# kento/TEZip

Measured on AMD Instinct MI355X. Metric: frames/sec (predict+delta-encode), 512x512 seq, higher is better.
Workload: dtype f32; 1 GPU; 512x512x3 synthetic turbulence stack, 80 frames per GPU (ONE 80-frame sequence), SWP 20-frame windows, warm_up 0, lossy rel 1e-3, entropy remap on; PredNet (3,48,96,192) glorot seed 123

## Files before the change

### tezip_amd/csrc/tz_conv_kernels.hip.h

```cpp
#pragma once
#include <type_traits>

#include "tz_internal.h"
#include "tz_math.hip.h"

typedef float f32x4 __attribute__((ext_vector_type(4)));

enum { EPI_RAW = 0, EPI_RELU = 1, EPI_LSTM = 2, EPI_LSTM_PACKED = 3, EPI_POOL_ERR = 4, EPI_LSTM3 = 5, EPI_RAW3 = 6 };

struct ConvSrc {
    const float* p;
    long long nstride;
    int C;
    int pstride;
    int up;
    int cpt;
};

struct ConvArgs {
    ConvSrc src[2];
    int nsrc;
    int H, W, tiles_x, tiles_y, ncb;
    const float* Wp;
    const float* Wimg;
// ... 1150 lines not shown

    __builtin_amdgcn_s_setprio(1);
    wait_vm_n(inflight);
    wg_barrier();
    {
        const float* pa = smem;
        const float* wb = smem + P0 * 256 + lane * NTI;
#pragma unroll
        for (int tap = 0; tap < 9; ++tap) {
            const int dy = tap / 3, dx = tap % 3;
            const int xo = MAP == MAP_PARITY ? (dx == 1 ? ((wcls & 1) ? 1 - PW / 2 : PW / 2) : (dx >> 1)) : dx;
            const int toff = 4 * (dy * PW + xo);
#pragma unroll
            for (int kk = 0; kk < KS0; ++kk) {
                float fa[MT];
#pragma unroll
                for (int mt = 0; mt < MT; ++mt) fa[mt] = pa[abase[mt] + toff + kk * 4 * NP16];
                mfma_step(fa, wb + (tap * KS0 + kk) * 64 * NTI);
            }
        }
    }
    if (UPS) {
#pragma unroll 1
        for (int b = 1; b < nblk; ++b) {
            if (b + 1 < nblk) {
                wg_barrier();
                inflight = issue_block(b + 1, (b + 1) & 1);
            } else {
                inflight = 0;
            }
            wait_vm_n(inflight);
            wg_barrier();
            const float* pa = smem + (b & 1) * BUFP * 256;
            const float* wb = pa + U16_PIECES * 256 + lane * NTI;
#pragma unroll
            for (int tap = 0; tap < 4; ++tap) {
                const int toff = 4 * ((tap >> 1) * LW + (tap & 1));
#pragma unroll
                for (int kk = 0; kk < 4; ++kk) {
                    float fa[MT];
#pragma unroll
                    for (int mt = 0; mt < MT; ++mt) fa[mt] = pa[abase_lo[mt] + toff + kk * 4 * NPU16];
                    mfma_step(fa, wb + ((tap * 4 + wcls) * 4 + kk) * 64 * NTI);
                }
            }
        }
    }
    __builtin_amdgcn_s_setprio(0);
    if (EPI == EPI_LSTM_PACKED) wg_barrier();
    if (EPI == EPI_POOL_ERR && a.dead_half) conv_epilogue<NT, EPI, MAP, true>(a, acc, n, cb, ty0, tx0, wv, lane, smem);
    else conv_epilogue<NT, EPI, MAP>(a, acc, n, cb, ty0, tx0, wv, lane, smem);
}

template <int CIN, int COUT>
__global__ __launch_bounds__(256) void k_conv_small(const ConvArgs a) {
    __shared__ float tile[PPIX * CIN];
    const int tid = threadIdx.x;
    const int ntiles = a.tiles_x * a.tiles_y;
    const int tileid = blockIdx.x % ntiles, n = blockIdx.x / ntiles;
    const int ty0 = (tileid / a.tiles_x) * 16, tx0 = (tileid % a.tiles_x) * 16;
    const float* base = a.src[0].p + (long long)n * a.src[0].nstride;
    for (int i = tid; i < PPIX * CIN; i += 256) {
        const int pp = i / CIN, ci = i - pp * CIN;
        const int yy = ty0 - 1 + pp / PW, xx = tx0 - 1 + pp % PW;
        tile[i] = (yy >= 0 && yy < a.H && xx >= 0 && xx < a.W) ? base[((long long)yy * a.W + xx) * CIN + ci] : 0.0f;
    }
    __syncthreads();
    const int py = tid >> 4, px = tid & 15;
    float acc[COUT];
#pragma unroll
    for (int co = 0; co < COUT; ++co) acc[co] = a.bias[co];
#pragma unroll
    for (int tap = 0; tap < 9; ++tap) {
        const float* x = tile + ((py + tap / 3) * PW + px + tap % 3) * CIN;
#pragma unroll
        for (int ci = 0; ci < CIN; ++ci)
#pragma unroll
            for (int co = 0; co < COUT; ++co) acc[co] = __builtin_fmaf(x[ci], a.Wp[(tap * 16 + ci) * a.ncols + co], acc[co]);
    }
    const int y = ty0 + py, xq = tx0 + px;
    if (y < a.H && xq < a.W) {
        const long long pix = (long long)y * a.W + xq;
        float* o = a.out0 + (long long)(a.out_idx ? a.out_idx[n] : n) * a.out0_nstride + pix * COUT;
        float v[COUT];
#pragma unroll
        for (int co = 0; co < COUT; ++co) {
            v[co] = tz_relu(acc[co]);
            if (a.clip1 && v[co] > 1.0f) v[co] = 1.0f;
            o[co] = v[co];
        }
        if (COUT == 3 && a.e0_out) {
            const int slot = a.e0_slot[n];
            if (slot >= 0 && a.dead_half) {
                float* e = a.e0_out + (long long)slot * a.e0_nstride + pix * 8;
                *(float4*)(e + 4) = make_float4(v[0], v[1], v[2], 0.0f);
            } else if (slot >= 0) {
                float d1[3], d2[3];
#pragma unroll
                for (int c = 0; c < 3; ++c) {
                    const float h = a.e0_ahat[pix * 3 + c];
                    d1[c] = h - v[c];
                    d2[c] = v[c] - h;
                }
                float* e = a.e0_out + (long long)slot * a.e0_nstride + pix * 8;
                *(float4*)e = make_float4(tz_relu(d1[0]), tz_relu(d1[1]), tz_relu(d1[2]), 0.0f);
                *(float4*)(e + 4) = make_float4(tz_relu(d2[0]), tz_relu(d2[1]), tz_relu(d2[2]), 0.0f);
            }
        }
    }
}

template <int MAP>
__global__ __launch_bounds__(256) void k_to_fragments(const float* __restrict__ src, int H, int W, int tiles_x, int tiles_y,
                                                      int ncols, int ncb, int NT, float* __restrict__ dst) {
    const long long total = (long long)tiles_x * tiles_y * ncb * 8 * MT * NT * 256;
    for (long long i = (long long)blockIdx.x * blockDim.x + threadIdx.x; i < total; i += (long long)gridDim.x * blockDim.x) {
        const int r = (int)(i & 3), lane = (int)((i >> 2) & 63);
        long long q = i >> 8;
        const int nt = (int)(q % NT); q /= NT;
        const int mt = (int)(q % MT); q /= MT;
        const int wv = (int)(q & 7); q >>= 3;
        const int cb = (int)(q % ncb);
        const int tile = (int)(q / ncb);
        int py, px;
        row_to_patch<MAP>(wv * 32 + mt * 16 + (lane >> 4) * 4 + r, py, px);
        const int y = (tile / tiles_x) * 16 + py, x = (tile % tiles_x) * 16 + px;
        dst[i] = (y < H && x < W) ? src[((long long)y * W + x) * ncols + cb * NT * 16 + nt * 16 + (lane & 15)] : 0.0f;
    }
}

__global__ __launch_bounds__(256) void k_uniform_ring(const unsigned* __restrict__ src, int H, int W, int ncols, int by_tile,
                                                      int* __restrict__ ring) {
    const unsigned* centre = src + ((size_t)(H / 2) * W + W / 2) * ncols;
    const int ry = ref_tile_origin(H), rx = ref_tile_origin(W);
    const unsigned total = (unsigned)H * (unsigned)W * (unsigned)ncols;
    int mine = 0;
    for (unsigned i = blockIdx.x * blockDim.x + threadIdx.x; i < total; i += gridDim.x * blockDim.x) {
        const unsigned pix = i / (unsigned)ncols, col = i - pix * (unsigned)ncols;
        const int y = (int)(pix / (unsigned)W), x = (int)(pix - (unsigned)y * (unsigned)W);
        const unsigned want = by_tile ? src[((size_t)(ry + (y & 15)) * W + rx + (x & 15)) * ncols + col] : centre[col];
        if (src[i] != want) {
            const int dy = y < H - 1 - y ? y : H - 1 - y, dx = x < W - 1 - x ? x : W - 1 - x;
            const int w = (dy < dx ? dy : dx) + 1;
            mine = w > mine ? w : mine;
        }
    }
#pragma unroll
    for (int o = 32; o >= 1; o >>= 1) {
        const int other = __shfl_xor(mine, o);
        mine = other > mine ? other : mine;
    }
    if ((threadIdx.x & 63) == 0 && mine) atomicMax(ring, mine);
}

__global__ __launch_bounds__(256) void k_live_blocks(const unsigned* __restrict__ src, long long npx, int C, int nblocks,
                                                     unsigned long long* __restrict__ live, unsigned mask = 0x7fffffffu) {
    const long long total = npx * C;
    unsigned long long mine = 0;
    for (long long i = (long long)blockIdx.x * blockDim.x + threadIdx.x; i < total; i += (long long)gridDim.x * blockDim.x) {
// ... 69 lines not shown
```

### tezip_amd/csrc/tz_l0_kernels.hip.h

```cpp
#pragma once
#include "tz_conv_kernels.hip.h"

typedef float f32x2 __attribute__((ext_vector_type(2)));

namespace tzl0 {

typedef const __attribute__((address_space(4))) f32x2* cpair;
__device__ __forceinline__ cpair as_const(const float* p) { return (cpair)(unsigned long long)p; }

__device__ __forceinline__ f32x2 fma2(float x, f32x2 w, f32x2 acc) { return __builtin_elementwise_fma((f32x2){x, x}, w, acc); }

__device__ __forceinline__ f32x2 zero2() {
    f32x2 z = {0.0f, 0.0f};
    asm volatile("" : "+v"(z));
    return z;
}

__device__ __forceinline__ float add_zero(float x) {
    float r;
    asm("v_add_f32 %0, 0, %1" : "=v"(r) : "v"(x));
    return r;
}

}

namespace tzl0 {
static constexpr int GT = 32;
static constexpr int EW = GT + 2;
static constexpr int RW = GT / 2 + 2;
static constexpr int RPIX = RW * RW;
static constexpr int R_ITEMS = (RPIX * 4 + 255) / 256;
template <int NP>
__device__ __forceinline__ constexpr int pair_col(int p) { return NP == 6 ? 2 * p : (p < 2 ? 2 * p : 2 * p + 2); }
template <int NP>
__device__ __forceinline__ float col_of(const f32x2 (&acc)[NP], int col) {
    return NP == 6 || col < 4 ? acc[col >> 1][col & 1] : acc[(col - 2) >> 1][col & 1];
}
}

template <bool DEAD0, int NP>
__global__ __launch_bounds__(256, DEAD0 && NP == 5 ? 4 : 3) void k_l0_gates(const ConvArgs a, const float* wg) {
    using namespace tzl0;
    constexpr int NQ = DEAD0 ? 1 : 2;
    constexpr int LDSQ = NQ * EW * EW > 16 * RPIX / 4 ? NQ * EW * EW : 16 * RPIX / 4;
    __shared__ f32x4 smem[LDSQ];
    float* const planes = (float*)smem;
    const int tid = threadIdx.x, lane = tid & 63, cls = __builtin_amdgcn_readfirstlane(tid >> 6);
    const int pa = cls >> 1, pb = cls & 1;
    const int tx32 = (a.W + GT - 1) / GT, ty32 = (a.H + GT - 1) / GT;
    const int tile = blockIdx.x % (tx32 * ty32), n = blockIdx.x / (tx32 * ty32);
    const int ty0 = (tile / tx32) * GT, tx0 = (tile % tx32) * GT;
    const int H2 = a.H >> 1, W2 = a.W >> 1;
    const int nub = a.src[1].cpt;

    const float* r1 = a.src[1].p + (long long)n * a.src[1].nstride;
    const int rps = a.src[1].pstride;
    f32x4 pre[R_ITEMS];
    auto fetch_r1 = [&](int b) {
#pragma unroll
        for (int k = 0; k < R_ITEMS; ++k) {
            const int i = tid + 256 * k, px = i >> 2, q = i & 3;
            const int Y = px / RW, X = px - Y * RW;
            const int ly = (ty0 >> 1) - 1 + Y, lx = (tx0 >> 1) - 1 + X;
            pre[k] = (f32x4){0.0f, 0.0f, 0.0f, 0.0f};
            if (px < RPIX && ly >= 0 && ly < H2 && lx >= 0 && lx < W2) pre[k] = *(const f32x4*)(r1 + ((long long)ly * W2 + lx) * rps + b * 16 + 4 * q);
        }
    };
    auto store_r1 = [&]() {
#pragma unroll
        for (int k = 0; k < R_ITEMS; ++k) {
            const int i = tid + 256 * k, px = i >> 2, q = i & 3;
            if (px < RPIX) {
#pragma unroll
                for (int c = 0; c < 4; ++c) planes[(4 * q + c) * RPIX + px] = pre[k][c];
            }
        }
    };
    if (nub > 0) fetch_r1(0);
    {
        const float* base = a.src[0].p + (long long)n * a.src[0].nstride;
        for (int i = tid; i < NQ * EW * EW; i += 256) {
            const int q = DEAD0 ? 1 : i / (EW * EW), slot = DEAD0 ? i : i - q * (EW * EW);
            const int y = slot / EW, x = slot - y * EW;
            const int yy = ty0 - 1 + y, xx = tx0 - 1 + x;
            f32x4 v = {0.0f, 0.0f, 0.0f, 0.0f};
            if (yy >= 0 && yy < a.H && xx >= 0 && xx < a.W) v = *(const f32x4*)(base + ((long long)yy * a.W + xx) * 8 + 4 * q);
            smem[i] = v;
        }
    }
    const int by = lane >> 2, bxg = lane & 3;
    const int y = ty0 + 2 * by + pa, x0 = tx0 + 8 * bxg + pb;
    f32x2 acc[4][NP];
#pragma unroll
    for (int k = 0; k < 4; ++k) {
        const int x = x0 + 2 * k;
        const long long pix = (y < a.H && x < a.W) ? (long long)y * a.W + x : 0;
#pragma unroll
        for (int p = 0; p < NP; ++p) acc[k][p] = *(const f32x2*)(a.init + pix * a.ncols + pair_col<NP>(p));
    }
    const f32x2 z = zero2();
    __syncthreads();
#pragma unroll
    for (int dy = 0; dy < 3; ++dy) {
        f32x4 xr[NQ][9];
#pragma unroll
        for (int q = 0; q < NQ; ++q)
#pragma unroll
            for (int j = 0; j < 9; ++j) xr[q][j] = smem[q * (EW * EW) + (2 * by + pa + dy) * EW + 8 * bxg + pb + j];
#pragma unroll
        for (int dx = 0; dx < 3; ++dx) {
            const int tap = dy * 3 + dx;
#pragma unroll
            for (int q = 0; q < NQ; ++q) {
#pragma unroll
                for (int ch = 0; ch < 3; ++ch) {
                    const float* wrow = a.Wp + (tap * 16 + 4 * (DEAD0 ? 1 : q) + ch) * a.ncols;
                    f32x2 w[NP];
#pragma unroll
                    for (int p = 0; p < NP; ++p) w[p] = as_const(wrow + pair_col<NP>(p))[0];
#pragma unroll
                    for (int k = 0; k < 4; ++k)
#pragma unroll
                        for (int p = 0; p < NP; ++p) acc[k][p] = fma2(xr[q][2 * k + dx][ch], w[p], acc[k][p]);
                }
#pragma unroll
                for (int k = 0; k < 4; ++k)
#pragma unroll
                    for (int p = 0; p < NP; ++p) acc[k][p] = acc[k][p] + z;
            }
        }
    }
    const float* xbase = planes + (by + pa) * RW + 4 * bxg + pb;
#pragma unroll 1
    for (int b = 0; b < nub; ++b) {
        __syncthreads();
        store_r1();
        __syncthreads();
        if (b + 1 < nub) fetch_r1(b + 1);
        const float* wblk = wg + (long long)(cls * nub + b) * (64 * 12);
        auto request = [&](int s, f32x2 (&w)[2][6], float (&xv)[2][4]) {
            const int tp = s >> 3, c0 = 2 * (s & 7);
            const cpair wrow = as_const(wblk + s * 24);
            const float* xp = xbase + c0 * RPIX + (tp >> 1) * RW + (tp & 1);
#pragma unroll
            for (int c = 0; c < 2; ++c) {
#pragma unroll
                for (int p = 0; p < 6; ++p) w[c][p] = wrow[6 * c + p];
#pragma unroll
                for (int k = 0; k < 4; ++k) xv[c][k] = xp[c * RPIX + k];
            }
        };
        auto landed = [&]() {
            __builtin_amdgcn_s_waitcnt(0xc07f);
            __builtin_amdgcn_sched_barrier(0);
        };
        auto compute = [&](const f32x2 (&w)[2][6], const float (&xv)[2][4]) {
#pragma unroll
            for (int c = 0; c < 2; ++c)
#pragma unroll
                for (int k = 0; k < 4; ++k)
#pragma unroll
                    for (int p = 0; p < NP; ++p) acc[k][p] = fma2(xv[c][k], w[c][pair_col<NP>(p) >> 1], acc[k][p]);
            __builtin_amdgcn_sched_barrier(0);
        };
        f32x2 wa[2][6], wb[2][6];
        float xa[2][4], xb[2][4];
        request(0, wa, xa);
        landed();
#pragma unroll 1
        for (int s = 0; s < 32; s += 2) {
            request(s + 1, wb, xb);
            compute(wa, xa);
            landed();
            request(s + 2, wa, xa);
            compute(wb, xb);
            landed();
        }
    }
    constexpr int R = 3;
    float* o0 = a.out0 + (long long)n * a.out0_nstride;
    float* o1 = a.out1 ? a.out1 + (long long)n * a.out1_nstride : nullptr;
#pragma unroll
    for (int k = 0; k < 4; ++k) {
        const int x = x0 + 2 * k;
        const bool ok = y < a.H && x < a.W;
        const long long pix = ok ? (long long)y * a.W + x : 0;
#pragma unroll
        for (int c = 0; c < R; ++c) {
            const float gi = tz_hard_sigmoid(col_of<NP>(acc[k], c));
            const float gg = tz_tanh(col_of<NP>(acc[k], 2 * R + c));
            const float go = tz_hard_sigmoid(col_of<NP>(acc[k], 3 * R + c));
            const float t2 = gi * gg;
            float cc;
            if (NP == 6) {
                const float gf = tz_hard_sigmoid(col_of<NP>(acc[k], R + c));
                const float cp = a.aux ? a.aux[pix * R + c] : 0.0f;
                const float t1 = gf * cp;
                cc = t1 + t2;
            } else {
                cc = add_zero(t2);
            }
            const float rr = go * tz_tanh(cc);
            if (ok) {
                o0[pix * R + c] = rr;
                if (o1) o1[pix * R + c] = cc;
            }
        }
    }
}
```

### tezip_amd/csrc/tz_prednet.hip

```cpp
#include <algorithm>
#include <atomic>
#include <cmath>

#include "tz_conv_kernels.hip.h"
#include "tz_wino_kernels.hip.h"
#include "tz_l0_kernels.hip.h"

struct Seg {
    int row_off, C;
    int up;
    int half = 0;
    int row(int c) const { return half && c >= half ? 4 + c - half : c; }
};
struct PackedConv {
    float* d_W = nullptr;
    float* d_Wimg = nullptr;
    float* d_Wblk = nullptr;
    float* d_Wblk0 = nullptr;
    bool pos_finite = false;
    std::vector<float> h_W0;
    float* d_Wlat = nullptr;
    float* d_Wwino = nullptr;
    float* d_Wwino2 = nullptr;
    const float* d_zero = nullptr;
    float* d_bias = nullptr;
    int nslots = 0, ncols = 0, NT = 1, ncb = 1;
    int wino_finite = 0;
    bool wino_all_finite = false;
    std::vector<Seg> segs;
};

enum { UNI_G0 = 0, UNI_C0 = 1, UNI_AHAT0 = 2 };
enum { UNI_USE_WINO_INIT = 1, UNI_USE_WINO_CELL = 2, UNI_USE_TILES = 4, UNI_USE_ALL = 7 };

struct tz_model {
    int L = 0;
    int stack[TZ_MAX_LEVELS] = {0}, rstack[TZ_MAX_LEVELS] = {0};
    std::vector<std::vector<float>> w;
    int Hp = 0, Wp = 0, maxB = 0;
    int cap = 0;
    bool prepared = false;
    float *R0[TZ_MAX_LEVELS] = {0}, *C0[TZ_MAX_LEVELS] = {0}, *Ahat0[TZ_MAX_LEVELS] = {0}, *G0[TZ_MAX_LEVELS] = {0};
    float *G0f[TZ_MAX_LEVELS] = {0}, *C0f[TZ_MAX_LEVELS] = {0};
    int ring[3][TZ_MAX_LEVELS] = {{0}};
    int tring[3][TZ_MAX_LEVELS] = {{0}};
    const float* uni[3][TZ_MAX_LEVELS] = {{0}};
    int uniform_mask = 0;
    int dead[TZ_MAX_LEVELS] = {0}, dead_gate[TZ_MAX_LEVELS] = {0}, dead_a[TZ_MAX_LEVELS] = {0};
    bool dead0 = false;
    bool dead0_hold = false;
    bool deadf[TZ_MAX_LEVELS] = {false};
    bool deadhalf[TZ_MAX_LEVELS] = {false};
    bool e0_dirty = false;
    bool l0valu_g = false, deadf0 = false;
    float* l0_wg = nullptr;
    float *E[TZ_MAX_LEVELS] = {0}, *R1[TZ_MAX_LEVELS] = {0};
    float* P[TZ_MAX_LEVELS] = {0};
    int Pcap[TZ_MAX_LEVELS] = {0};
    std::vector<signed char> epart_choice;
    PackedConv a_conv[TZ_MAX_LEVELS], gate_t1[TZ_MAX_LEVELS], ahat0_t1;
    PackedConv gate_nf[TZ_MAX_LEVELS];
    float* d_zero = nullptr;
    int e0s = 0;
    int* d_idx = nullptr;
    std::vector<void*> allocs;
    const float* a_k(int l) const { return w[2 * l].data(); }
    const float* a_b(int l) const { return w[2 * l + 1].data(); }
    const float* ahat_k(int l) const { return w[2 * (L - 1) + 2 * l].data(); }
    const float* ahat_b(int l) const { return w[2 * (L - 1) + 2 * l + 1].data(); }
    int gate_base(int g) const {
        static const int pos[4] = {2, 1, 0, 3};
        return 2 * (L - 1) + 2 * L + pos[g] * 2 * L;
    }
    const float* g_k(int g, int l) const { return w[gate_base(g) + 2 * l].data(); }
    const float* g_b(int g, int l) const { return w[gate_base(g) + 2 * l + 1].data(); }
    int gate_cin(int l) const { return rstack[l] + 2 * stack[l] + (l < L - 1 ? rstack[l + 1] : 0); }
};

static int dmalloc(tz_ctx* ctx, tz_model* m, void** p, size_t bytes) {
    if (bytes == 0) bytes = 16;
    hipError_t e = hipMalloc(p, bytes);
    if (e != hipSuccess) return tz_fail(ctx, TZ_ERR_NOMEM, "hipMalloc(%zu) failed: %s", bytes, hipGetErrorString(e));
    m->allocs.push_back(*p);
    return tz_poison(ctx, *p, bytes);
}

// ... 378 lines not shown
        return tz_fail(ctx, TZ_ERR_INVALID, "tz_set_contract: %d is not 0 (by frame size), 1 (TZ-PA1) or 2 (TZ-PA2)", contract);
    ctx->contract = contract;
    return TZ_OK;
}
extern "C" int tz_get_contract(tz_ctx* ctx) { return ctx ? effective_contract(ctx) : TZ_ERR_INVALID; }

extern "C" int tz_set_conv_impl(tz_ctx* ctx, int lds_dma) {
    if (!ctx) return TZ_ERR_INVALID;
    if (lds_dma < 0 || lds_dma > 5 || (lds_dma >> 1) > 2)
        return tz_fail(ctx, TZ_ERR_INVALID, "tz_set_conv_impl: %d is not 0 / 1 (+ 2 = never k_convlat, + 4 = k_convlat wherever eligible)", lds_dma);
    ctx->conv_impl = (lds_dma & 1) ? 1 : 0;
    const int lat = lds_dma >> 1;
    ctx->lat_mode = lat == 1 ? 0 : (lat == 2 ? 2 : 1);
    return TZ_OK;
}

struct LatPlan {
    bool use, wide;
    int blocks;
};
static LatPlan lat_plan(const tz_ctx* ctx, int NT, int epi, bool ups, bool fullk, const ConvArgs& a, int nbatch) {
    LatPlan lp = {false, false, 0};
    if (!(a.Wlat && a.nsrc > 0 && fullk && ctx->conv_impl && ctx->lat_mode && (NT == 3 || NT == 4) &&
          (epi == EPI_POOL_ERR || (epi == EPI_LSTM && NT == 4))))
        return lp;
    const int ts_ = (epi != EPI_POOL_ERR && ups) ? 8 : 4;
    const long long wg16 = (long long)a.ncb * a.tiles_x * a.tiles_y * nbatch;
    const long long rows_ = (a.H + ts_ - 1) / ts_ * (ts_ == 8 ? 4 : 1);
    const long long wglat1 = (long long)a.ncb * ((a.W + ts_ - 1) / ts_) * rows_ * nbatch;
    const long long wglat2 = (long long)a.ncb * ((a.W + 2 * ts_ - 1) / (2 * ts_)) * rows_ * nbatch;
    static const long long wide_min = getenv("TEZIP_LAT_WIDE_MIN") ? atoll(getenv("TEZIP_LAT_WIDE_MIN")) : 2560;
    lp.wide = wglat1 > wide_min;
    int slots = 0;
    for (int s = 0; s < a.nsrc; ++s) slots += a.src[s].cpt * (a.src[s].up ? 4 : 9);
    const double t16 = slots * 1.08 * (double)((wg16 + 255) / 256);
    const double per_slot = lp.wide ? 0.134 * (double)((wglat2 + 255) / 256) : std::max(0.105, 0.078 * (double)((wglat1 + 255) / 256));
    const double tlat = slots * per_slot * (ts_ == 8 ? 1.1 : 1.0) + 2.5;
    lp.use = wg16 <= 768 && (ctx->lat_mode == 2 || tlat < 0.9 * t16);
    lp.blocks = (int)(lp.wide ? wglat2 : wglat1);
    return lp;
}

static int launch_conv(tz_ctx* ctx, int NT, int epi, const ConvArgs& a, int nbatch, int wino_dead = 0, const float* wino3 = nullptr,
                       const float* wino3q = nullptr) {
    tz_prof_scope ps(ctx, TZP_CONV);
    bool ups = false, fullk = true;
    for (int s = 0; s < a.nsrc; ++s) {
        ups = ups || a.src[s].up;
        fullk = fullk && (a.src[s].C % 16) == 0;
        const long long hs = a.src[s].up ? a.H >> 1 : a.H, ws = a.src[s].up ? a.W >> 1 : a.W;
        fullk = fullk && hs * ws * a.src[s].pstride * 4 < (1LL << 32);
    }
    ps.sub = TZP_CONV_GEN;
    if (epi == EPI_RELU && a.nsrc == 1 && !ups && a.src[0].C == 3 && a.Cout == 3 && ctx->conv_impl) {
        ps.sub = TZP_CONV_SMALL;
        hipLaunchKernelGGL((k_conv_small<3, 3>), dim3(a.tiles_x * a.tiles_y * nbatch), dim3(256), 0, ctx->stream, a);
        TZ_HIP(ctx, hipGetLastError());
        return TZ_OK;
    }
    if (const tz_model* m = ctx->model; m && ctx->conv_impl && a.nsrc > 0 && a.src[0].pstride == 8) {
        if (m->l0valu_g && a.Wblk0 && epi == EPI_LSTM_PACKED && ups && a.nsrc == 2 && a.init && a.Wp == m->gate_t1[0].d_W) {
            ps.sub = TZP_CONV16B;
            const int blocks = ((a.W + tzl0::GT - 1) / tzl0::GT) * ((a.H + tzl0::GT - 1) / tzl0::GT) * nbatch;
            hipLaunchKernelGGL((k_l0_gates<true, 5>), dim3(blocks), dim3(256), 0, ctx->stream, a, m->l0_wg);
            TZ_HIP(ctx, hipGetLastError());
            return TZ_OK;
        }
    }
    if (a.Wblk && a.nsrc > 0 && !a.src[0].up && a.src[0].pstride == 8 && ctx->conv_impl) {
        const int blocks = a.ncb * a.tiles_x * a.tiles_y * nbatch;
#define TZ_CASE16B(nt, e, u)                                                                                    \
    if (NT == nt && epi == e && ups == u) {                                                                     \
        ps.sub = TZP_CONV16B;                                                                                   \
        if (a.Wblk0) hipLaunchKernelGGL((k_conv16b<nt, e, u, true>), dim3(blocks), dim3(NTHR), 0, ctx->stream, a); \
        else hipLaunchKernelGGL((k_conv16b<nt, e, u>), dim3(blocks), dim3(NTHR), 0, ctx->stream, a);            \
        TZ_HIP(ctx, hipGetLastError());                                                                         \
        return TZ_OK;                                                                                           \
    }
        TZ_CASE16B(1, EPI_LSTM_PACKED, true) TZ_CASE16B(1, EPI_LSTM_PACKED, false)
        TZ_CASE16B(1, EPI_POOL_ERR, false) TZ_CASE16B(3, EPI_POOL_ERR, false) TZ_CASE16B(4, EPI_POOL_ERR, false)
#undef TZ_CASE16B
    }
    if (a.Wwino && effective_contract(ctx) == 2 && fullk && (epi == EPI_LSTM || epi == EPI_POOL_ERR || epi == EPI_RAW)) {
        ps.sub = TZP_WINO;
        return launch_wino(ctx, NT, epi, ups, a, nbatch, false, wino_dead, wino3, wino3q);
    }
    {
        const LatPlan lp = lat_plan(ctx, NT, epi, ups, fullk, a, nbatch);
        if (!lp.use) goto no_lat;
        const bool wide = lp.wide;
        const int blocks = lp.blocks;
        ps.sub = TZP_CONVLAT;
#define TZ_LAT(e, u)                                                                                          \
    do {                                                                                                      \
        if (wide) hipLaunchKernelGGL((k_convlat<e, u, 2>), dim3(blocks), dim3(256), 0, ctx->stream, a);       \
        else hipLaunchKernelGGL((k_convlat<e, u, 1>), dim3(blocks), dim3(256), 0, ctx->stream, a);            \
    } while (0)
        if (epi == EPI_LSTM && ups) TZ_LAT(EPI_LSTM, true);
        else if (epi == EPI_LSTM) TZ_LAT(EPI_LSTM, false);
        else TZ_LAT(EPI_POOL_ERR, false);
#undef TZ_LAT
        TZ_HIP(ctx, hipGetLastError());
        return TZ_OK;
    }
no_lat:
    if (a.Wimg && a.nsrc > 0 && fullk && ctx->conv_impl) {
#define TZ_CASE16(nt, e, u)                          \
    if (NT == nt && epi == e && ups == u) {          \
        ps.sub = TZP_CONV16;                         \
        launch_conv16_t<nt, e, u>(ctx, a, nbatch);   \
        TZ_HIP(ctx, hipGetLastError());              \
        return TZ_OK;                                \
    }
        TZ_CASE16(4, EPI_LSTM, false) TZ_CASE16(4, EPI_LSTM, true)
        TZ_CASE16(3, EPI_POOL_ERR, false) TZ_CASE16(4, EPI_POOL_ERR, false)
#undef TZ_CASE16
    }
// ... 240 lines not shown
    const char* env = getenv("TEZIP_DEADF");
    const bool on = !env || atoi(env) != 0;
    const bool log = getenv("TEZIP_DEADF_LOG") && atoi(getenv("TEZIP_DEADF_LOG"));
    unsigned long long h_live[TZ_MAX_LEVELS] = {0};
    for (int l = 0; l < TZ_MAX_LEVELS; ++l) m->deadf[l] = false;
    if (!on && !log) return TZ_OK;
    {
        unsigned long long* d_live = nullptr;
        TZ_TRY(dmalloc(ctx, m, (void**)&d_live, sizeof(h_live)));
        TZ_HIP(ctx, hipMemsetAsync(d_live, 0, sizeof(h_live), ctx->stream));
        for (int l = 1; l < L; ++l) {
            const long long nwords = (long long)(m->Hp >> l) * (m->Wp >> l) * m->rstack[l];
            hipLaunchKernelGGL(k_live_blocks, dim3((unsigned)std::min<long long>((nwords + 255) / 256, 4096)), dim3(256), 0, ctx->stream,
                               (const unsigned*)m->C0[l], nwords, 1, 1, d_live + l, 0xffffffffu);
            TZ_HIP(ctx, hipGetLastError());
        }
        TZ_HIP(ctx, hipMemcpyAsync(h_live, d_live, sizeof(h_live), hipMemcpyDeviceToHost, ctx->stream));
        TZ_HIP(ctx, hipStreamSynchronize(ctx->stream));
    }
    for (int l = 1; l < L; ++l) {
        const bool zero = !(h_live[l] & 1);
        const bool form = m->gate_t1[l].d_Wwino && m->gate_t1[l].NT == 4;
        const bool finite = form && m->gate_t1[l].wino_all_finite;
        m->deadf[l] = on && zero && form && finite;
        if (m->deadf[l]) {
            std::vector<ColSrc> cols, cols3;
            int NT;
            TZ_TRY(gate_cols(ctx, m, l, &cols, &NT));
            for (size_t c = 0; c < cols.size(); ++c)
                if ((c % 64) / 16 != 1) cols3.push_back(cols[c]);
            TZ_TRY(pack_wino(ctx, m, m->gate_t1[l].segs, cols3, 3, &m->gate_nf[l]));
            m->deadf[l] = m->gate_nf[l].d_Wwino != nullptr;
        }
        if (log)
            fprintf(stderr, "[tezip] dead forget gate, level %d: C0 +0 everywhere: %s, forget-gate columns left out: %s%s\n", l, zero ? "yes" : "no",
                    m->deadf[l] ? "yes" : "no",
                    m->deadf[l] ? " (3 of 4 column tiles in every k_wino gate launch, fused or split)"
                    : !zero     ? ""
                    : !on       ? " (TEZIP_DEADF=0)"
                    : !form     ? " (no k_wino form)"
                                : " (a weight of the convolution is not finite)");
    }
    return TZ_OK;
}

static int choose_l0_forms(tz_ctx* ctx, tz_model* m) {
    const char* env = getenv("TEZIP_L0VALU");
    const bool on = !env || atoi(env) != 0;
    const bool log = getenv("TEZIP_L0VALU_LOG") && atoi(getenv("TEZIP_L0VALU_LOG"));
    m->l0valu_g = m->deadf0 = false;
    m->l0_wg = nullptr;
    const bool shape = m->L > 1 && m->stack[0] == 3 && m->rstack[0] == 3 && m->e0s == 8 && m->rstack[1] % 16 == 0;
    const PackedConv& pg = m->gate_t1[0];
    const bool form_g = shape && pg.d_Wblk && pg.NT == 1 && pg.ncols == 16 && pg.segs.size() == 2;
    bool zero = false, finite = false;
    if (on && form_g) {
        unsigned long long h_live = 0, *d_live = nullptr;
        TZ_TRY(dmalloc(ctx, m, (void**)&d_live, sizeof(h_live)));
        TZ_HIP(ctx, hipMemsetAsync(d_live, 0, sizeof(h_live), ctx->stream));
        const long long nwords = (long long)m->Hp * m->Wp * m->rstack[0];
        hipLaunchKernelGGL(k_live_blocks, dim3((unsigned)std::min<long long>((nwords + 255) / 256, 4096)), dim3(256), 0, ctx->stream,
                           (const unsigned*)m->C0[0], nwords, 1, 1, d_live, 0xffffffffu);
        TZ_HIP(ctx, hipGetLastError());
        TZ_HIP(ctx, hipMemcpyAsync(&h_live, d_live, sizeof(h_live), hipMemcpyDeviceToHost, ctx->stream));
        TZ_HIP(ctx, hipStreamSynchronize(ctx->stream));
        zero = !(h_live & 1);
        std::vector<float> W((size_t)pg.nslots * 16 * pg.ncols);
        TZ_HIP(ctx, hipMemcpy(W.data(), pg.d_W, W.size() * 4, hipMemcpyDeviceToHost));
        finite = true;
        for (float v : W) finite = finite && std::isfinite(v);
        const int nub = pg.segs[1].C / 16;
        std::vector<float> G((size_t)4 * nub * 64 * 12 + 24, 0.0f);
        for (int cls = 0; cls < 4; ++cls)
            for (int b = 0; b < nub; ++b)
                for (int tp = 0; tp < 4; ++tp)
                    for (int ch = 0; ch < 16; ++ch)
                        for (int c = 0; c < 12; ++c)
                            G[((((size_t)cls * nub + b) * 4 + tp) * 16 + ch) * 12 + c] = W[((size_t)(9 + 16 * b + 4 * tp + cls) * 16 + ch) * pg.ncols + c];
        TZ_TRY(dmalloc(ctx, m, (void**)&m->l0_wg, G.size() * 4));
        TZ_HIP(ctx, hipMemcpy(m->l0_wg, G.data(), G.size() * 4, hipMemcpyHostToDevice));
        const char* envf = getenv("TEZIP_DEADF");
        m->deadf0 = zero && finite && (!envf || atoi(envf) != 0);
        m->l0valu_g = m->deadf0 && pg.d_Wblk0 != nullptr;
    }
    if (log) {
        fprintf(stderr, "[tezip] level 0 A: k_conv16b (its vector-ALU form was not faster: EXPERIMENTS.md)\n");
        fprintf(stderr, "[tezip] level 0 gates: %s%s\n", m->l0valu_g ? "k_l0_gates (vector ALU)" : "k_conv16b",
                m->l0valu_g   ? ", forget-gate columns left out: yes (9 of 12 gate columns)"
                : !on         ? " (TEZIP_L0VALU=0)"
                : !form_g     ? " (not the reference shape)"
                : !pg.d_Wblk0 ? " (the positive half of E_0 is walked: k_conv16b is the faster form)"
                : !zero       ? " (the forget gate is needed: k_conv16b is the faster form)"
                : !finite     ? " (a weight of the convolution is not finite: the forget gate is needed)"
                              : " (TEZIP_DEADF=0: the forget gate is kept)");
    }
    return TZ_OK;
}

static int choose_wino_forms(tz_ctx* ctx, tz_model* m) {
    const char* env = getenv("TEZIP_WINO2Q");
    const bool on = !env || atoi(env) != 0;
    const bool log = getenv("TEZIP_WINO2Q_LOG") && atoi(getenv("TEZIP_WINO2Q_LOG"));
    for (int l = 1; l < m->L; ++l)
        for (int k = 0; k < 2; ++k) {
            if (k == 1 && l == m->L - 1) continue;
            PackedConv& pc = k == 0 ? (m->deadf[l] ? m->gate_nf[l] : m->gate_t1[l]) : m->a_conv[l];
            pc.d_Wwino2 = nullptr;
// ... 307 lines not shown
                    TZ_TRY(epart_measure(ctx, n, d_idx, stride, d_frames_u8, H, W, d_in_stack, d_out_stack, slot0, d_next_slot, &choice));
                    m->epart_choice[n] = (signed char)choice;
                    skip_err0 = false;
                    err0_keys_only = false;
                }
            }
            use = m->epart_choice[n] == 1;
        }
    }
    return predict_batch_impl(ctx, n, d_idx, stride, d_frames_u8, H, W, d_in_stack, d_out_stack, slot0, d_next_slot, skip_err0, fused_next,
                              err0_keys_only, use);
}

static int predict_batch_impl(tz_ctx* ctx, int n, const int* d_idx, int stride, const uint8_t* d_frames_u8, int H, int W,
                              const float* d_in_stack, float* d_out_stack, int slot0, const int* d_next_slot, bool skip_err0,
                              bool* fused_next, bool err0_keys_only, bool use_epart) {
    tz_model* m = ctx->model;
    const int L = m->L, Hp = m->Hp, Wp = m->Wp;
    auto hl = [&](int l) { return Hp >> l; };
    auto wl = [&](int l) { return Wp >> l; };
    auto npx = [&](int l) { return (long long)hl(l) * wl(l); };
    if (fused_next) *fused_next = false;
    if (!skip_err0) {
        tz_prof_scope ps(ctx, TZP_ERR0);
        int gx = (int)std::min<long long>((npx(0) + 255) / 256, 2048);
        hipLaunchKernelGGL(k_err0, dim3(gx, n), dim3(256), 0, ctx->stream, d_frames_u8, H, W, d_in_stack, d_idx,
                           d_idx + stride, m->Ahat0[0], Hp, Wp, m->stack[0], m->e0s, m->E[0] + (long long)slot0 * npx(0) * m->e0s,
                           err0_keys_only ? 1 : 0);
        TZ_HIP(ctx, hipGetLastError());
    }
    auto set_uniform = [&](const float*& u, int& ring, int& tring, int k, int l, int use) {
        const bool on = (m->uniform_mask & use) && m->ring[k][l] >= 0;
        u = on ? m->uni[k][l] : nullptr;
        ring = on ? m->ring[k][l] : -1;
        tring = (m->uniform_mask & use) ? m->tring[k][l] : -1;
    };
    auto gate_args = [&](int l, ConvArgs& a) {
        const PackedConv& pc = m->gate_t1[l];
        memset(&a, 0, sizeof(a));
        const int ec = l == 0 ? m->e0s : 2 * m->stack[l];
        long long ns[2] = {npx(l) * ec, l < L - 1 ? npx(l + 1) * m->rstack[l + 1] : 0};
        const float* ptrs[2] = {m->E[l] + slot0 * ns[0], l < L - 1 ? m->R1[l + 1] + slot0 * ns[1] : nullptr};
        fill_srcs(a, pc, ptrs, ns, ec);
        if (m->dead0_hold) a.Wblk0 = nullptr;
        set_geom(a, hl(l), wl(l));
        a.init = m->G0[l];
        a.initf = m->G0f[l];
        a.Cout = m->rstack[l];
        a.R = m->rstack[l];
        a.aux = m->C0[l];
        a.auxf = m->C0f[l];
        a.out0_nstride = npx(l) * m->rstack[l];
        a.out0 = m->R1[l] + slot0 * a.out0_nstride;
        set_uniform(a.init_u, a.init_ring, a.init_tring, UNI_G0, l, l >= 1 ? UNI_USE_WINO_INIT : 0);
        set_uniform(a.aux_u, a.aux_ring, a.aux_tring, UNI_C0, l, l >= 1 ? UNI_USE_WINO_CELL : 0);
    };
    auto aconv_args = [&](int l, ConvArgs& a) {
        const PackedConv& pc = m->a_conv[l];
        memset(&a, 0, sizeof(a));
        const int ec = l == 0 ? m->e0s : 2 * m->stack[l];
        long long ns[2] = {npx(l) * ec, 0};
        const float* ptrs[2] = {m->E[l] + slot0 * ns[0], nullptr};
        fill_srcs(a, pc, ptrs, ns, ec);
        if (m->dead0_hold) a.Wblk0 = nullptr;
        set_geom(a, hl(l), wl(l));
        a.Cout = m->stack[l + 1];
        a.aux = m->Ahat0[l + 1];
        a.init_tring = a.aux_tring = -1;
        a.out0_nstride = npx(l + 1) * 2 * m->stack[l + 1];
        a.out0 = m->E[l + 1] + slot0 * a.out0_nstride;
        a.dead_half = m->deadhalf[l + 1];
    };
    bool epart[TZ_MAX_LEVELS] = {false};
    if (use_epart) {
        double idle;
        epart_levels(ctx, m, n, epart, &idle);
    }
    auto wino3 = [&](int l) -> const float* { return m->deadf[l] ? m->gate_nf[l].d_Wwino : nullptr; };
    auto wino3q = [&](int l) -> const float* { return m->deadf[l] ? m->gate_nf[l].d_Wwino2 : nullptr; };
    auto pcols = [&](int l) { return m->deadf[l] ? 3 * m->rstack[l] : m->gate_t1[l].ncols; };
    auto epart_launch = [&](int l) -> int {
        if (!ctx->ev_epart_src[l]) {
            TZ_HIP(ctx, hipEventCreateWithFlags(&ctx->ev_epart_src[l], hipEventDisableTiming));
            TZ_HIP(ctx, hipEventCreateWithFlags(&ctx->ev_epart_done[l], hipEventDisableTiming));
        }
        ConvArgs ge;
        gate_args(l, ge);
        ge.wino_stride = (ge.src[0].C + ge.src[1].C) >> 2;
        ge.wino_first = 0;
        ge.nsrc = 1;
        ge.initf = nullptr;
        ge.aux = ge.auxf = nullptr;
        ge.aux_u = nullptr;
        ge.aux_ring = ge.aux_tring = -1;
        ge.out0_nstride = npx(l) * pcols(l);
        ge.out0 = m->P[l] + slot0 * ge.out0_nstride;
        ge.ipw = 1;
        TZ_HIP(ctx, hipEventRecord(ctx->ev_epart_src[l], ctx->stream));
        TZ_HIP(ctx, hipStreamWaitEvent(ctx->stream2, ctx->ev_epart_src[l], 0));
        hipStream_t main_stream = ctx->stream;
        ctx->stream = ctx->stream2;
        int rc = launch_conv(ctx, 4, EPI_RAW, ge, n, m->dead_gate[l], wino3(l), wino3q(l));
        ctx->stream = main_stream;
        TZ_TRY(rc);
        TZ_HIP(ctx, hipEventRecord(ctx->ev_epart_done[l], ctx->stream2));
        return TZ_OK;
    };
// ... 222 lines not shown
```

Before: 3490 frames/s.

## Rework small conv and layer-0 gate kernels for register reuse and packed FMA

k_conv_small now drops the LDS staging and has each thread compute four adjacent pixels from f32x4 row loads held in registers, with scalar-cached weights and vectorized stores. k_l0_gates is specialized to the dead-forget-gate form and computes only the 9 live gate columns using v_pk_fma_f32 with op_sel to pick scalar weights. It also moves inputs into per-channel padded LDS planes with a new pixel interleave, and takes a uniform-init fast path for interior tiles. These changes cut redundant loads and wasted FMA columns, at the cost of inline asm complexity and new alignment assumptions.

```diff
diff --git a/tezip_amd/csrc/tz_conv_kernels.hip.h b/tezip_amd/csrc/tz_conv_kernels.hip.h
--- a/tezip_amd/csrc/tz_conv_kernels.hip.h
+++ b/tezip_amd/csrc/tz_conv_kernels.hip.h
@@ -1226,59 +1226,112 @@
     else conv_epilogue<NT, EPI, MAP>(a, acc, n, cb, ty0, tx0, wv, lane, smem);
 }
 
+static constexpr int CS_TW = 64, CS_TH = 16;
+static constexpr int CS_G = CS_TW / 4;
+__host__ __device__ __forceinline__ int conv_small_tiles(int H, int W) { return ((W + CS_TW - 1) / CS_TW) * ((H + CS_TH - 1) / CS_TH); }
+
 template <int CIN, int COUT>
 __global__ __launch_bounds__(256) void k_conv_small(const ConvArgs a) {
-    __shared__ float tile[PPIX * CIN];
+    static_assert(CIN == 3 && COUT == 3, "the one shape launch_conv sends here");
+    typedef const __attribute__((address_space(4))) float* cfloat;
+    typedef const __attribute__((address_space(4))) int* cint;
     const int tid = threadIdx.x;
-    const int ntiles = a.tiles_x * a.tiles_y;
+    const int tsx = (a.W + CS_TW - 1) / CS_TW, ntiles = conv_small_tiles(a.H, a.W);
     const int tileid = blockIdx.x % ntiles, n = blockIdx.x / ntiles;
-    const int ty0 = (tileid / a.tiles_x) * 16, tx0 = (tileid % a.tiles_x) * 16;
+    const int ty0 = (tileid / tsx) * CS_TH, tx0 = (tileid % tsx) * CS_TW;
     const float* base = a.src[0].p + (long long)n * a.src[0].nstride;
-    for (int i = tid; i < PPIX * CIN; i += 256) {
-        const int pp = i / CIN, ci = i - pp * CIN;
-        const int yy = ty0 - 1 + pp / PW, xx = tx0 - 1 + pp % PW;
-        tile[i] = (yy >= 0 && yy < a.H && xx >= 0 && xx < a.W) ? base[((long long)yy * a.W + xx) * CIN + ci] : 0.0f;
-    }
-    __syncthreads();
-    const int py = tid >> 4, px = tid & 15;
-    float acc[COUT];
-#pragma unroll
-    for (int co = 0; co < COUT; ++co) acc[co] = a.bias[co];
-#pragma unroll
-    for (int tap = 0; tap < 9; ++tap) {
-        const float* x = tile + ((py + tap / 3) * PW + px + tap % 3) * CIN;
-#pragma unroll
-        for (int ci = 0; ci < CIN; ++ci)
-#pragma unroll
-            for (int co = 0; co < COUT; ++co) acc[co] = __builtin_fmaf(x[ci], a.Wp[(tap * 16 + ci) * a.ncols + co], acc[co]);
-    }
-    const int y = ty0 + py, xq = tx0 + px;
-    if (y < a.H && xq < a.W) {
-        const long long pix = (long long)y * a.W + xq;
-        float* o = a.out0 + (long long)(a.out_idx ? a.out_idx[n] : n) * a.out0_nstride + pix * COUT;
-        float v[COUT];
-#pragma unroll
-        for (int co = 0; co < COUT; ++co) {
-            v[co] = tz_relu(acc[co]);
-            if (a.clip1 && v[co] > 1.0f) v[co] = 1.0f;
-            o[co] = v[co];
-        }
-        if (COUT == 3 && a.e0_out) {
-            const int slot = a.e0_slot[n];
+    const int py = tid / CS_G, g = tid % CS_G;
+    const int y = ty0 + py, x = tx0 + 4 * g;
+    if (y >= a.H || x >= a.W) return;
+    f32x4 xr[3][5];
+#pragma unroll
+    for (int ky = 0; ky < 3; ++ky) {
+        const int yy = y - 1 + ky;
+#pragma unroll
+        for (int q = 0; q < 5; ++q) xr[ky][q] = (f32x4){0.0f, 0.0f, 0.0f, 0.0f};
+        if (yy >= 0 && yy < a.H) {
+            const f32x4* r = (const f32x4*)(base + ((long long)yy * a.W + x) * 3);
+            if (x > 0) xr[ky][0] = r[-1];
+#pragma unroll
+            for (int q = 1; q < 4; ++q) xr[ky][q] = r[q - 1];
+            if (x + 4 < a.W) xr[ky][4] = r[3];
+        }
+    }
+    const cfloat bias = (cfloat)(unsigned long long)a.bias;
+    float acc[4][3];
+#pragma unroll
+    for (int p = 0; p < 4; ++p)
+#pragma unroll
+        for (int co = 0; co < 3; ++co) acc[p][co] = bias[co];
+    unsigned long long wnext = (unsigned long long)a.Wp;
+#pragma unroll
+    for (int ky = 0; ky < 3; ++ky) {
+        const cfloat wp = (cfloat)wnext;
+#pragma unroll
+        for (int kx = 0; kx < 3; ++kx) {
+#pragma unroll
+            for (int ci = 0; ci < 3; ++ci) {
+#pragma unroll
+                for (int co = 0; co < 3; ++co) {
+                    const float w = wp[(kx * 16 + ci) * 16 + co];
+#pragma unroll
+                    for (int p = 0; p < 4; ++p) {
+                        const int k = 1 + 3 * (p + kx) + ci;
+                        acc[p][co] = __builtin_fmaf(xr[ky][k >> 2][k & 3], w, acc[p][co]);
+                    }
+                }
+            }
+            if (kx == 0 && ky < 2) {
+                wnext = (unsigned long long)(a.Wp + (ky + 1) * 3 * 16 * 16);
+                asm volatile("" : "+s"(wnext), "+v"(acc[0][0]), "+v"(acc[0][1]), "+v"(acc[0][2]), "+v"(acc[1][0]), "+v"(acc[1][1]), "+v"(acc[1][2]),
+                             "+v"(acc[2][0]), "+v"(acc[2][1]), "+v"(acc[2][2]), "+v"(acc[3][0]), "+v"(acc[3][1]), "+v"(acc[3][2]));
+            }
+        }
+    }
+    {
+        const long long pix = (long long)y * a.W + x;
+        const int frame = a.out_idx ? ((cint)(unsigned long long)a.out_idx)[n] : n;
+        float* o = a.out0 + (long long)frame * a.out0_nstride + pix * 3;
+        float v[4][3];
+#pragma unroll
+        for (int p = 0; p < 4; ++p)
+#pragma unroll
+            for (int co = 0; co < 3; ++co) {
+                v[p][co] = tz_relu(acc[p][co]);
+                if (a.clip1 && v[p][co] > 1.0f) v[p][co] = 1.0f;
+            }
+        if (((unsigned long long)o & 15) == 0) {
+            f32x4* o4 = (f32x4*)o;
+            o4[0] = (f32x4){v[0][0], v[0][1], v[0][2], v[1][0]};
+            o4[1] = (f32x4){v[1][1], v[1][2], v[2][0], v[2][1]};
+            o4[2] = (f32x4){v[2][2], v[3][0], v[3][1], v[3][2]};
+        } else {
+#pragma unroll
+            for (int p = 0; p < 4; ++p)
+#pragma unroll
+                for (int co = 0; co < 3; ++co) o[p * 3 + co] = v[p][co];
+        }
+        if (a.e0_out) {
+            const int slot = ((cint)(unsigned long long)a.e0_slot)[n];
+            float* e = a.e0_out + (long long)(slot >= 0 ? slot : 0) * a.e0_nstride + pix * 8;
             if (slot >= 0 && a.dead_half) {
-                float* e = a.e0_out + (long long)slot * a.e0_nstride + pix * 8;
-                *(float4*)(e + 4) = make_float4(v[0], v[1], v[2], 0.0f);
+#pragma unroll
+                for (int p = 0; p < 4; ++p) *(f32x4*)(e + 8 * p + 4) = (f32x4){v[p][0], v[p][1], v[p][2], 0.0f};
             } else if (slot >= 0) {
-                float d1[3], d2[3];
-#pragma unroll
-                for (int c = 0; c < 3; ++c) {
-                    const float h = a.e0_ahat[pix * 3 + c];
-                    d1[c] = h - v[c];
-                    d2[c] = v[c] - h;
-                }
-                float* e = a.e0_out + (long long)slot * a.e0_nstride + pix * 8;
-                *(float4*)e = make_float4(tz_relu(d1[0]), tz_relu(d1[1]), tz_relu(d1[2]), 0.0f);
-                *(float4*)(e + 4) = make_float4(tz_relu(d2[0]), tz_relu(d2[1]), tz_relu(d2[2]), 0.0f);
+                const f32x4* h4 = (const f32x4*)(a.e0_ahat + pix * 3);
+                const f32x4 h[3] = {h4[0], h4[1], h4[2]};
+#pragma unroll
+                for (int p = 0; p < 4; ++p) {
+                    float d1[3], d2[3];
+#pragma unroll
+                    for (int c = 0; c < 3; ++c) {
+                        const float hv = h[(3 * p + c) >> 2][(3 * p + c) & 3];
+                        d1[c] = hv - v[p][c];
+                        d2[c] = v[p][c] - hv;
+                    }
+                    *(f32x4*)(e + 8 * p) = (f32x4){tz_relu(d1[0]), tz_relu(d1[1]), tz_relu(d1[2]), 0.0f};
+                    *(f32x4*)(e + 8 * p + 4) = (f32x4){tz_relu(d2[0]), tz_relu(d2[1]), tz_relu(d2[2]), 0.0f};
+                }
             }
         }
     }
diff --git a/tezip_amd/csrc/tz_l0_kernels.hip.h b/tezip_amd/csrc/tz_l0_kernels.hip.h
--- a/tezip_amd/csrc/tz_l0_kernels.hip.h
+++ b/tezip_amd/csrc/tz_l0_kernels.hip.h
@@ -8,7 +8,11 @@
 typedef const __attribute__((address_space(4))) f32x2* cpair;
 __device__ __forceinline__ cpair as_const(const float* p) { return (cpair)(unsigned long long)p; }
 
-__device__ __forceinline__ f32x2 fma2(float x, f32x2 w, f32x2 acc) { return __builtin_elementwise_fma((f32x2){x, x}, w, acc); }
+__device__ __forceinline__ f32x2 fma2(f32x2 x, f32x2 w, int h, f32x2 acc) {
+    if (h) asm("v_pk_fma_f32 %0, %1, %2, %0 op_sel:[0,1,0] op_sel_hi:[1,1,1]" : "+v"(acc) : "v"(x), "s"(w));
+    else asm("v_pk_fma_f32 %0, %1, %2, %0 op_sel:[0,0,0] op_sel_hi:[1,0,1]" : "+v"(acc) : "v"(x), "s"(w));
+    return acc;
+}
 
 __device__ __forceinline__ f32x2 zero2() {
     f32x2 z = {0.0f, 0.0f};
@@ -22,29 +26,27 @@
     return r;
 }
 
-}
-
-namespace tzl0 {
 static constexpr int GT = 32;
 static constexpr int EW = GT + 2;
+static constexpr int EPL = EW * EW;
 static constexpr int RW = GT / 2 + 2;
 static constexpr int RPIX = RW * RW;
+static constexpr int RS = 20;
+static constexpr int RPL = RW * RS + 2;
 static constexpr int R_ITEMS = (RPIX * 4 + 255) / 256;
-template <int NP>
-__device__ __forceinline__ constexpr int pair_col(int p) { return NP == 6 ? 2 * p : (p < 2 ? 2 * p : 2 * p + 2); }
-template <int NP>
-__device__ __forceinline__ float col_of(const f32x2 (&acc)[NP], int col) {
-    return NP == 6 || col < 4 ? acc[col >> 1][col & 1] : acc[(col - 2) >> 1][col & 1];
-}
-}
-
-template <bool DEAD0, int NP>
-__global__ __launch_bounds__(256, DEAD0 && NP == 5 ? 4 : 3) void k_l0_gates(const ConvArgs a, const float* wg) {
+static constexpr int NC = 9;
+static constexpr int NCOLS = 16;
+__device__ __forceinline__ constexpr int gate_col(int c) { return c < 3 ? c : c + 3; }
+
+__device__ __forceinline__ bool tile32_uniform(const float* u, int ring, int y0, int x0, int H, int W) {
+    return u && ring >= 0 && y0 >= ring && y0 + GT <= H - ring && x0 >= ring && x0 + GT <= W - ring;
+}
+}
+
+__global__ __launch_bounds__(256, 4) void k_l0_gates(const ConvArgs a, const float* wg) {
     using namespace tzl0;
-    constexpr int NQ = DEAD0 ? 1 : 2;
-    constexpr int LDSQ = NQ * EW * EW > 16 * RPIX / 4 ? NQ * EW * EW : 16 * RPIX / 4;
-    __shared__ f32x4 smem[LDSQ];
-    float* const planes = (float*)smem;
+    constexpr int LDSF = 3 * EPL > 16 * RPL ? 3 * EPL : 16 * RPL;
+    __shared__ float planes[LDSF];
     const int tid = threadIdx.x, lane = tid & 63, cls = __builtin_amdgcn_readfirstlane(tid >> 6);
     const int pa = cls >> 1, pb = cls & 1;
     const int tx32 = (a.W + GT - 1) / GT, ty32 = (a.H + GT - 1) / GT;
@@ -70,67 +72,83 @@
 #pragma unroll
         for (int k = 0; k < R_ITEMS; ++k) {
             const int i = tid + 256 * k, px = i >> 2, q = i & 3;
+            const int Y = px / RW, X = px - Y * RW;
             if (px < RPIX) {
 #pragma unroll
-                for (int c = 0; c < 4; ++c) planes[(4 * q + c) * RPIX + px] = pre[k][c];
+                for (int c = 0; c < 4; ++c) planes[(4 * q + c) * RPL + Y * RS + X] = pre[k][c];
             }
         }
     };
     if (nub > 0) fetch_r1(0);
     {
         const float* base = a.src[0].p + (long long)n * a.src[0].nstride;
-        for (int i = tid; i < NQ * EW * EW; i += 256) {
-            const int q = DEAD0 ? 1 : i / (EW * EW), slot = DEAD0 ? i : i - q * (EW * EW);
-            const int y = slot / EW, x = slot - y * EW;
+        for (int i = tid; i < EPL; i += 256) {
+            const int y = i / EW, x = i - y * EW;
             const int yy = ty0 - 1 + y, xx = tx0 - 1 + x;
             f32x4 v = {0.0f, 0.0f, 0.0f, 0.0f};
-            if (yy >= 0 && yy < a.H && xx >= 0 && xx < a.W) v = *(const f32x4*)(base + ((long long)yy * a.W + xx) * 8 + 4 * q);
-            smem[i] = v;
+            if (yy >= 0 && yy < a.H && xx >= 0 && xx < a.W) v = *(const f32x4*)(base + ((long long)yy * a.W + xx) * 8 + 4);
+#pragma unroll
+            for (int ch = 0; ch < 3; ++ch) planes[ch * EPL + i] = v[ch];
         }
     }
     const int by = lane >> 2, bxg = lane & 3;
-    const int y = ty0 + 2 * by + pa, x0 = tx0 + 8 * bxg + pb;
-    f32x2 acc[4][NP];
-#pragma unroll
-    for (int k = 0; k < 4; ++k) {
-        const int x = x0 + 2 * k;
-        const long long pix = (y < a.H && x < a.W) ? (long long)y * a.W + x : 0;
-#pragma unroll
-        for (int p = 0; p < NP; ++p) acc[k][p] = *(const f32x2*)(a.init + pix * a.ncols + pair_col<NP>(p));
+    const int y = ty0 + 2 * by + pa, x0 = tx0 + 2 * bxg + pb;
+    f32x2 acc[2][NC];
+    if (tile32_uniform(a.init_u, a.init_ring, ty0, tx0, a.H, a.W)) {
+        const cpair row = as_const(a.init_u);
+#pragma unroll
+        for (int c = 0; c < NC; ++c) {
+            const float s = row[gate_col(c) >> 1][gate_col(c) & 1];
+            acc[0][c] = acc[1][c] = (f32x2){s, s};
+        }
+    } else {
+#pragma unroll
+        for (int k = 0; k < 4; ++k) {
+            const int x = x0 + 8 * k;
+            const long long pix = (y < a.H && x < a.W) ? (long long)y * a.W + x : 0;
+            const float* g = a.init + pix * NCOLS;
+            const f32x4 v0 = *(const f32x4*)g, v2 = *(const f32x4*)(g + 8);
+            const f32x2 v1 = *(const f32x2*)(g + 6);
+            const float col[NC] = {v0[0], v0[1], v0[2], v1[0], v1[1], v2[0], v2[1], v2[2], v2[3]};
+#pragma unroll
+            for (int c = 0; c < NC; ++c) acc[k >> 1][c][k & 1] = col[c];
+        }
     }
     const f32x2 z = zero2();
     __syncthreads();
 #pragma unroll
     for (int dy = 0; dy < 3; ++dy) {
-        f32x4 xr[NQ][9];
-#pragma unroll
-        for (int q = 0; q < NQ; ++q)
-#pragma unroll
-            for (int j = 0; j < 9; ++j) xr[q][j] = smem[q * (EW * EW) + (2 * by + pa + dy) * EW + 8 * bxg + pb + j];
+        f32x2 xe[3][3][2];
+#pragma unroll
+        for (int ch = 0; ch < 3; ++ch) {
+            const float* xp = planes + ch * EPL + (2 * by + pa + dy) * EW + 2 * bxg + pb;
+#pragma unroll
+            for (int dx = 0; dx < 3; ++dx)
+#pragma unroll
+                for (int pp = 0; pp < 2; ++pp) xe[ch][dx][pp] = (f32x2){xp[dx + 16 * pp], xp[dx + 16 * pp + 8]};
+        }
 #pragma unroll
         for (int dx = 0; dx < 3; ++dx) {
             const int tap = dy * 3 + dx;
 #pragma unroll
-            for (int q = 0; q < NQ; ++q) {
-#pragma unroll
-                for (int ch = 0; ch < 3; ++ch) {
-                    const float* wrow = a.Wp + (tap * 16 + 4 * (DEAD0 ? 1 : q) + ch) * a.ncols;
-                    f32x2 w[NP];
-#pragma unroll
-                    for (int p = 0; p < NP; ++p) w[p] = as_const(wrow + pair_col<NP>(p))[0];
-#pragma unroll
-                    for (int k = 0; k < 4; ++k)
-#pragma unroll
-                        for (int p = 0; p < NP; ++p) acc[k][p] = fma2(xr[q][2 * k + dx][ch], w[p], acc[k][p]);
-                }
-#pragma unroll
-                for (int k = 0; k < 4; ++k)
-#pragma unroll
-                    for (int p = 0; p < NP; ++p) acc[k][p] = acc[k][p] + z;
-            }
-        }
-    }
-    const float* xbase = planes + (by + pa) * RW + 4 * bxg + pb;
+            for (int ch = 0; ch < 3; ++ch) {
+                const cpair wrow = as_const(a.Wp + (tap * 16 + 4 + ch) * NCOLS);
+                f32x2 w[6];
+#pragma unroll
+                for (int p = 0; p < 6; ++p)
+                    if (p != 2) w[p] = wrow[p];
+#pragma unroll
+                for (int pp = 0; pp < 2; ++pp)
+#pragma unroll
+                    for (int c = 0; c < NC; ++c) acc[pp][c] = fma2(xe[ch][dx][pp], w[gate_col(c) >> 1], gate_col(c) & 1, acc[pp][c]);
+            }
+#pragma unroll
+            for (int pp = 0; pp < 2; ++pp)
+#pragma unroll
+                for (int c = 0; c < NC; ++c) acc[pp][c] = acc[pp][c] + z;
+        }
+    }
+    const float* xbase = planes + (by + pa) * RS + bxg + pb;
 #pragma unroll 1
     for (int b = 0; b < nub; ++b) {
         __syncthreads();
@@ -138,33 +156,34 @@
         __syncthreads();
         if (b + 1 < nub) fetch_r1(b + 1);
         const float* wblk = wg + (long long)(cls * nub + b) * (64 * 12);
-        auto request = [&](int s, f32x2 (&w)[2][6], float (&xv)[2][4]) {
+        auto request = [&](int s, f32x2 (&w)[2][6], f32x2 (&xv)[2][2]) {
             const int tp = s >> 3, c0 = 2 * (s & 7);
             const cpair wrow = as_const(wblk + s * 24);
-            const float* xp = xbase + c0 * RPIX + (tp >> 1) * RW + (tp & 1);
+            const float* xp = xbase + c0 * RPL + (tp >> 1) * RS + (tp & 1);
 #pragma unroll
             for (int c = 0; c < 2; ++c) {
 #pragma unroll
-                for (int p = 0; p < 6; ++p) w[c][p] = wrow[6 * c + p];
-#pragma unroll
-                for (int k = 0; k < 4; ++k) xv[c][k] = xp[c * RPIX + k];
+                for (int p = 0; p < 6; ++p)
+                    if (p != 2) w[c][p] = wrow[6 * c + p];
+#pragma unroll
+                for (int pp = 0; pp < 2; ++pp) xv[c][pp] = (f32x2){xp[c * RPL + 8 * pp], xp[c * RPL + 8 * pp + 4]};
             }
         };
         auto landed = [&]() {
             __builtin_amdgcn_s_waitcnt(0xc07f);
             __builtin_amdgcn_sched_barrier(0);
         };
-        auto compute = [&](const f32x2 (&w)[2][6], const float (&xv)[2][4]) {
+        auto compute = [&](const f32x2 (&w)[2][6], const f32x2 (&xv)[2][2]) {
 #pragma unroll
             for (int c = 0; c < 2; ++c)
 #pragma unroll
-                for (int k = 0; k < 4; ++k)
-#pragma unroll
-                    for (int p = 0; p < NP; ++p) acc[k][p] = fma2(xv[c][k], w[c][pair_col<NP>(p) >> 1], acc[k][p]);
+                for (int pp = 0; pp < 2; ++pp)
+#pragma unroll
+                    for (int col = 0; col < NC; ++col) acc[pp][col] = fma2(xv[c][pp], w[c][gate_col(col) >> 1], gate_col(col) & 1, acc[pp][col]);
             __builtin_amdgcn_sched_barrier(0);
         };
         f32x2 wa[2][6], wb[2][6];
-        float xa[2][4], xb[2][4];
+        f32x2 xa[2][2], xb[2][2];
         request(0, wa, xa);
         landed();
 #pragma unroll 1
@@ -182,24 +201,15 @@
     float* o1 = a.out1 ? a.out1 + (long long)n * a.out1_nstride : nullptr;
 #pragma unroll
     for (int k = 0; k < 4; ++k) {
-        const int x = x0 + 2 * k;
+        const int x = x0 + 8 * k;
         const bool ok = y < a.H && x < a.W;
         const long long pix = ok ? (long long)y * a.W + x : 0;
 #pragma unroll
         for (int c = 0; c < R; ++c) {
-            const float gi = tz_hard_sigmoid(col_of<NP>(acc[k], c));
-            const float gg = tz_tanh(col_of<NP>(acc[k], 2 * R + c));
-            const float go = tz_hard_sigmoid(col_of<NP>(acc[k], 3 * R + c));
-            const float t2 = gi * gg;
-            float cc;
-            if (NP == 6) {
-                const float gf = tz_hard_sigmoid(col_of<NP>(acc[k], R + c));
-                const float cp = a.aux ? a.aux[pix * R + c] : 0.0f;
-                const float t1 = gf * cp;
-                cc = t1 + t2;
-            } else {
-                cc = add_zero(t2);
-            }
+            const float gi = tz_hard_sigmoid(acc[k >> 1][c][k & 1]);
+            const float gg = tz_tanh(acc[k >> 1][R + c][k & 1]);
+            const float go = tz_hard_sigmoid(acc[k >> 1][2 * R + c][k & 1]);
+            const float cc = add_zero(gi * gg);
             const float rr = go * tz_tanh(cc);
             if (ok) {
                 o0[pix * R + c] = rr;
diff --git a/tezip_amd/csrc/tz_prednet.hip b/tezip_amd/csrc/tz_prednet.hip
--- a/tezip_amd/csrc/tz_prednet.hip
+++ b/tezip_amd/csrc/tz_prednet.hip
@@ -31,7 +31,7 @@
 };
 
 enum { UNI_G0 = 0, UNI_C0 = 1, UNI_AHAT0 = 2 };
-enum { UNI_USE_WINO_INIT = 1, UNI_USE_WINO_CELL = 2, UNI_USE_TILES = 4, UNI_USE_ALL = 7 };
+enum { UNI_USE_WINO_INIT = 1, UNI_USE_WINO_CELL = 2, UNI_USE_TILES = 4, UNI_USE_L0_INIT = 8, UNI_USE_ALL = 15 };
 
 struct tz_model {
     int L = 0;
@@ -516,17 +516,17 @@
         fullk = fullk && hs * ws * a.src[s].pstride * 4 < (1LL << 32);
     }
     ps.sub = TZP_CONV_GEN;
-    if (epi == EPI_RELU && a.nsrc == 1 && !ups && a.src[0].C == 3 && a.Cout == 3 && ctx->conv_impl) {
+    if (epi == EPI_RELU && a.nsrc == 1 && !ups && a.src[0].C == 3 && a.Cout == 3 && a.ncols == 16 && ctx->conv_impl) {
         ps.sub = TZP_CONV_SMALL;
-        hipLaunchKernelGGL((k_conv_small<3, 3>), dim3(a.tiles_x * a.tiles_y * nbatch), dim3(256), 0, ctx->stream, a);
+        hipLaunchKernelGGL((k_conv_small<3, 3>), dim3(conv_small_tiles(a.H, a.W) * nbatch), dim3(256), 0, ctx->stream, a);
         TZ_HIP(ctx, hipGetLastError());
         return TZ_OK;
     }
     if (const tz_model* m = ctx->model; m && ctx->conv_impl && a.nsrc > 0 && a.src[0].pstride == 8) {
-        if (m->l0valu_g && a.Wblk0 && epi == EPI_LSTM_PACKED && ups && a.nsrc == 2 && a.init && a.Wp == m->gate_t1[0].d_W) {
+        if (m->l0valu_g && a.Wblk0 && epi == EPI_LSTM_PACKED && ups && a.nsrc == 2 && a.init && a.ncols == tzl0::NCOLS && a.Wp == m->gate_t1[0].d_W) {
             ps.sub = TZP_CONV16B;
             const int blocks = ((a.W + tzl0::GT - 1) / tzl0::GT) * ((a.H + tzl0::GT - 1) / tzl0::GT) * nbatch;
-            hipLaunchKernelGGL((k_l0_gates<true, 5>), dim3(blocks), dim3(256), 0, ctx->stream, a, m->l0_wg);
+            hipLaunchKernelGGL(k_l0_gates, dim3(blocks), dim3(256), 0, ctx->stream, a, m->l0_wg);
             TZ_HIP(ctx, hipGetLastError());
             return TZ_OK;
         }
@@ -873,7 +873,7 @@
     m->l0_wg = nullptr;
     const bool shape = m->L > 1 && m->stack[0] == 3 && m->rstack[0] == 3 && m->e0s == 8 && m->rstack[1] % 16 == 0;
     const PackedConv& pg = m->gate_t1[0];
-    const bool form_g = shape && pg.d_Wblk && pg.NT == 1 && pg.ncols == 16 && pg.segs.size() == 2;
+    const bool form_g = shape && pg.d_Wblk && pg.NT == 1 && pg.ncols == tzl0::NCOLS && pg.segs.size() == 2;
     bool zero = false, finite = false;
     if (on && form_g) {
         unsigned long long h_live = 0, *d_live = nullptr;
@@ -1287,7 +1287,7 @@
         a.auxf = m->C0f[l];
         a.out0_nstride = npx(l) * m->rstack[l];
         a.out0 = m->R1[l] + slot0 * a.out0_nstride;
-        set_uniform(a.init_u, a.init_ring, a.init_tring, UNI_G0, l, l >= 1 ? UNI_USE_WINO_INIT : 0);
+        set_uniform(a.init_u, a.init_ring, a.init_tring, UNI_G0, l, l >= 1 ? UNI_USE_WINO_INIT : UNI_USE_L0_INIT);
         set_uniform(a.aux_u, a.aux_ring, a.aux_tring, UNI_C0, l, l >= 1 ? UNI_USE_WINO_CELL : 0);
     };
     auto aconv_args = [&](int l, ConvArgs& a) {
```

Result: faster. 3546 frames/s (median of 6 runs) (+1.6%).
